# adwardlee/multitask-end-to-end-video-captioning

Hardware: AMD Instinct MI355X
Metric: sampled caption tokens/sec (REINFORCE step) (higher is better)
Workload: dtype f32

## Files before the change

### include/s2vt.h

```cpp
#ifndef S2VT_H
#define S2VT_H

#include <stddef.h>
#include <stdint.h>

#ifdef __cplusplus
extern "C" {
#endif

#define S2VT_OK 0
#define S2VT_E_BADARG (-1)
#define S2VT_E_ALIGN (-2)
#define S2VT_E_WORKSPACE (-3)
#define S2VT_E_HIP (-4)
#define S2VT_E_CHAIN_TIMEOUT (-5)

typedef void* s2vt_stream;

typedef struct s2vt_dims {
    int32_t dim_image;
    int32_t n_words;
    int32_t word_dim;
    int32_t lstm_dim;
    int32_t n_video_lstm_step;
// ... 236 lines not shown
int s2vt_cast_bf16_split(const float* src, int32_t ld, const int32_t* rowidx, int32_t R, int32_t C, int32_t transpose, uint16_t* dst,
                         uint16_t* dst_lo, int32_t ldd, int32_t Rp, float* colsum, uint16_t* row_dst, uint16_t* row_dst_lo, int32_t row_ldd,
                         void* scratch, size_t scratch_bytes, s2vt_stream stream);
int s2vt_gemm_bf16x3_nt(const uint16_t* Ah, const uint16_t* Al, int32_t lda, const uint16_t* Bh, const uint16_t* Bl, int32_t ldb, float* C,
                        int32_t ldc, int32_t M, int32_t N, int32_t Kp, int32_t accumulate, void* scratch, size_t scratch_bytes, s2vt_stream stream);
int s2vt_gemm_bf16x3_nt_tile(const uint16_t* Ah, const uint16_t* Al, int32_t lda, const uint16_t* Bh, const uint16_t* Bl, int32_t ldb, float* C,
                             int32_t ldc, int32_t M, int32_t N, int32_t Kp, int32_t accumulate, s2vt_stream stream, int32_t tile);
int s2vt_gemm_bf16x3_nt_tile_choice(int32_t M, int32_t N, int32_t cus);
int s2vt_gemm_bf16x1_nt(const uint16_t* Ah, int32_t lda, const uint16_t* Bh, int32_t ldb, float* C, int32_t ldc, int32_t M, int32_t N, int32_t Kp,
                        int32_t accumulate, s2vt_stream stream);

int s2vt_gemm_bf16x3_tn(const uint16_t* Ah, const uint16_t* Al, int32_t lda, const uint16_t* Bh, const uint16_t* Bl, int32_t ldb, float* C,
                        int32_t ldc, int32_t M, int32_t N, int32_t K, int32_t accumulate, float* bias, void* scratch, size_t scratch_bytes,
                        s2vt_stream stream);
int s2vt_split_grad_active(int32_t N);
int s2vt_split_grad_dlogits_planes(const s2vt_dims* d, int32_t B, int32_t N, size_t* hi_offset, size_t* lo_offset, int32_t* ld);
int s2vt_softmax_nll_fwd_bwd_split(float* logits, int32_t ld, int32_t R, int32_t V, const int32_t* target, const float* coef, float smoothing,
                                   const float* smoothing_rows, float* nll, float* lp_target, const s2vt_dims* d, int32_t B, int32_t N,
                                   void* split_ws, size_t split_ws_bytes, s2vt_stream stream);

int s2vt_gemm_bf16x3_nn(const uint16_t* Ah, const uint16_t* Al, int32_t lda, const uint16_t* Bh, const uint16_t* Bl, int32_t ldb, float* C,
                        int32_t ldc, int32_t M, int32_t N, int32_t K, int32_t accumulate, const float* bias, void* scratch, size_t scratch_bytes,
                        s2vt_stream stream);

int s2vt_split_fwd_stage(void);
int s2vt_split_fwd_active(int32_t N);
int s2vt_teacher_forced_fwd_split(const s2vt_dims* d, const s2vt_params* p, const float* video, int32_t B, int32_t N,
                                  const int32_t* caption, int32_t caption_steps, const int32_t* live_rows, int32_t n_live, float keep,
                                  uint64_t seed, const int32_t* video_id, const int32_t* sample_id, float* logits_out,
                                  void* workspace, size_t workspace_bytes, const void* sampler_workspace,
                                  size_t sampler_workspace_bytes, int32_t sampler_rows, void* split_ws, size_t split_ws_bytes,
                                  s2vt_stream stream);

int s2vt_bptt_dvideo(const s2vt_dims* d, const s2vt_params* p, int32_t B, int32_t N, float* d_video, void* workspace,
                      size_t workspace_bytes, s2vt_stream stream);

int s2vt_embed_scatter_add(const float* dE, int32_t ld, const int32_t* idx, int32_t R, int32_t E, float* dWemb,
                           s2vt_stream stream);
int s2vt_embed_scatter_add2(const float* dE, int32_t ld, const int32_t* idx_a, const int32_t* idx_b, float scale, int32_t R, int32_t E,
                            float* dWemb, s2vt_stream stream);
int s2vt_embed_scatter_addk(const float* dE, int32_t ld, const int32_t* ids, const float* w, int32_t k, int32_t R, int32_t E, float* dWemb,
                            s2vt_stream stream);

int s2vt_caption_mask(const int32_t* ids, int32_t N, int32_t Tc, float* mask, int32_t* target_tm, float* mask_sum, float* mask_sum_copy, s2vt_stream stream);
int s2vt_pg_coef(const float* mask, const float* rewards, const float* baseline, float scale, int32_t N, int32_t Tc, float* coef_tm,
                 s2vt_stream stream);
// ... 223 lines not shown
```

### multitask-end-to-end-video-captioning_amd/_lib.py

```python
from __future__ import annotations

import ctypes as C
import os

_HERE = os.path.dirname(os.path.abspath(__file__))
_LIB = None


class S2VTLibraryError(RuntimeError):
    pass


class S2VTChainTimeout(S2VTLibraryError):
    """A persistent recurrence (csrc/chain.hip) was starved of CUs and gave up a grid-wide wait (S2VT_E_CHAIN_TIMEOUT):
    activations computed since are suspect, variable updates queued behind it were skipped on the device.  Recover with
    Video_Caption_Generator.recover() (synchronise, acknowledge, fall back to per-step launches) and repeat the step."""


MODEL_RESIDUAL = 1


class Dims(C.Structure):
    _fields_ = [(n, C.c_int32) for n in ("dim_image", "n_words", "word_dim", "lstm_dim", "n_video_lstm_step",
                                         "n_caption_lstm_step", "label_dim", "reserved")]
# ... 99 lines not shown
    "s2vt_beam_workspace_bytes": (_sz, [_DP, _i32, _i32]),
    "s2vt_beam_encode": (C.c_int, [_DP, _PP, _vp, _i32, _i32, _vp, _sz, _vp]),
    "s2vt_beam_step": (C.c_int, [_DP, _PP, _i32, _i32, _i32, _i32, _vp, _vp, _vp, _i32, _vp, _vp, _vp, _vp, _sz, _vp]),
    "s2vt_train_workspace_bytes": (_sz, [_DP, _i32, _i32]),
    "s2vt_teacher_forced_fwd": (C.c_int, [_DP, _PP, _vp, _i32, _i32, _vp, _f32, _u64, _vp, _vp, _vp, _vp, _sz, _vp]),
    "s2vt_teacher_forced_fwd_reuse": (C.c_int, [_DP, _PP, _vp, _i32, _i32, _vp, _f32, _u64, _vp, _vp, _vp, _vp, _sz, _vp, _sz, _i32, _vp]),
    "s2vt_gemm_nt_splitk": (C.c_int, [_vp, _i32, _vp, _i32, _vp, _i32, _i32, _i32, _i32, _i32, _i32, _vp, _sz, _vp]),
    "s2vt_teacher_forced_fwd_steps": (C.c_int, [_DP, _PP, _vp, _i32, _i32, _vp, _i32, _f32, _u64, _vp, _vp, _vp, _vp, _sz, _vp, _sz, _i32, _vp]),
    "s2vt_teacher_forced_fwd_live": (C.c_int, [_DP, _PP, _vp, _i32, _i32, _vp, _i32, _vp, _i32, _f32, _u64, _vp, _vp, _vp, _vp, _sz, _vp, _sz, _i32, _vp]),
    "s2vt_bptt_bwd_live": (C.c_int, [_DP, _PP, _PP, _vp, _i32, _i32, _vp, _i32, _vp, _i32, _f32, _u64, _vp, _vp, _vp, _sz, _i32, _vp]),
    "s2vt_bf16_grad_workspace_bytes": (_sz, [_DP, _i32, _i32]),
    "s2vt_bptt_bwd_bf16": (C.c_int, [_DP, _PP, _PP, _vp, _i32, _i32, _vp, _i32, _vp, _i32, _f32, _u64, _vp, _vp, _vp, _sz, _i32, _vp, _sz, _vp]),
    "s2vt_cast_bf16": (C.c_int, [_vp, _i32, _vp, _i32, _i32, _i32, _vp, _i32, _i32, _vp, _vp, _i32, _vp, _sz, _vp]),
    "s2vt_gemm_bf16_nt": (C.c_int, [_vp, _i32, _vp, _i32, _vp, _i32, _i32, _i32, _i32, _i32, _i32, _vp]),
    "s2vt_split_grad_workspace_bytes": (_sz, [_DP, _i32, _i32]),
    "s2vt_bptt_bwd_split": (C.c_int, [_DP, _PP, _PP, _vp, _i32, _i32, _vp, _i32, _vp, _i32, _f32, _u64, _vp, _vp, _vp, _sz, _i32, _vp, _sz, _vp]),
    "s2vt_cast_bf16_split": (C.c_int, [_vp, _i32, _vp, _i32, _i32, _i32, _vp, _vp, _i32, _i32, _vp, _vp, _vp, _i32, _vp, _sz, _vp]),
    "s2vt_gemm_bf16x3_nt": (C.c_int, [_vp, _vp, _i32, _vp, _vp, _i32, _vp, _i32, _i32, _i32, _i32, _i32, _vp, _sz, _vp]),
    "s2vt_gemm_bf16x3_nt_tile": (C.c_int, [_vp, _vp, _i32, _vp, _vp, _i32, _vp, _i32, _i32, _i32, _i32, _i32, _vp, _i32]),
    "s2vt_gemm_bf16x3_nt_tile_choice": (C.c_int, [_i32, _i32, _i32]),
    "s2vt_gemm_bf16x1_nt": (C.c_int, [_vp, _i32, _vp, _i32, _vp, _i32, _i32, _i32, _i32, _i32, _vp]),
    "s2vt_gemm_bf16x3_tn": (C.c_int, [_vp, _vp, _i32, _vp, _vp, _i32, _vp, _i32, _i32, _i32, _i32, _i32, _vp, _vp, _sz, _vp]),
    "s2vt_gemm_bf16x3_nn": (C.c_int, [_vp, _vp, _i32, _vp, _vp, _i32, _vp, _i32, _i32, _i32, _i32, _i32, _vp, _vp, _sz, _vp]),
    "s2vt_split_grad_active": (C.c_int, [_i32]),
    "s2vt_split_fwd_stage": (C.c_int, []),
    "s2vt_split_fwd_active": (C.c_int, [_i32]),
    "s2vt_teacher_forced_fwd_split": (C.c_int, [_DP, _PP, _vp, _i32, _i32, _vp, _i32, _vp, _i32, _f32, _u64, _vp, _vp, _vp, _vp, _sz, _vp, _sz, _i32,
                                                _vp, _sz, _vp]),
    "s2vt_train_workspace_dz2": (C.c_int, [_DP, _i32, _i32, C.POINTER(_sz), C.POINTER(_sz)]),
    "s2vt_split_grad_dlogits_planes": (C.c_int, [_DP, _i32, _i32, C.POINTER(_sz), C.POINTER(_sz), C.POINTER(_i32)]),
    "s2vt_softmax_nll_fwd_bwd_split": (C.c_int, [_vp, _i32, _i32, _i32, _vp, _vp, _f32, _vp, _vp, _vp, _DP, _i32, _i32, _vp, _sz, _vp]),
    "s2vt_bptt_bwd_steps": (C.c_int, [_DP, _PP, _PP, _vp, _i32, _i32, _vp, _i32, _f32, _u64, _vp, _vp, _vp, _sz, _i32, _vp]),
    "s2vt_softmax_nll_fwd_bwd": (C.c_int, [_vp, _i32, _i32, _i32, _vp, _vp, _f32, _vp, _vp, _vp]),
    "s2vt_softmax_unshifted_argmax": (C.c_int, [_vp, _i32, _i32, _i32, _vp, _vp, _vp]),
    "s2vt_softmax_nll_fwd_bwd_rows": (C.c_int, [_vp, _i32, _i32, _i32, _vp, _vp, _vp, _vp, _vp, _vp]),
    "s2vt_bptt_bwd": (C.c_int, [_DP, _PP, _PP, _vp, _i32, _i32, _vp, _f32, _u64, _vp, _vp, _vp, _sz, _vp]),
    "s2vt_bptt_bwd_phase": (C.c_int, [_DP, _PP, _PP, _vp, _i32, _i32, _vp, _f32, _u64, _vp, _vp, _vp, _sz, _i32, _vp]),
    "s2vt_bptt_dvideo": (C.c_int, [_DP, _PP, _i32, _i32, _vp, _vp, _sz, _vp]),
    "s2vt_embed_scatter_add": (C.c_int, [_vp, _i32, _vp, _i32, _i32, _vp, _vp]),
    "s2vt_caption_mask": (C.c_int, [_vp, _i32, _i32, _vp, _vp, _vp, _vp, _vp]),
    "s2vt_pg_coef": (C.c_int, [_vp, _vp, _vp, _f32, _i32, _i32, _vp, _vp]),
    "s2vt_xe_prep": (C.c_int, [_vp, _vp, _i32, _i32, _f32, _f32, _i32, _vp, _vp, _vp, _vp]),
    "s2vt_mixed_prep": (C.c_int, [_vp, _vp, _vp, _vp, _vp, _vp, _i32, _i32, _i32, C.c_double, _f32, _i32, _f32, _f32, _vp, _vp, _vp, _vp, _vp, _vp]),
    "s2vt_mixed_loss": (C.c_int, [_vp, _vp, _vp, _i64, _i32, _i32, _vp, _vp]),
    "s2vt_step_scalars": (C.c_int, [_vp, _vp, _i64, _vp, _vp, _vp, _vp, _vp, _vp]),
    "s2vt_grad_finalize": (C.c_int, [_vp, _vp, _i64, _vp, _f32, _vp, _vp]),
# ... 127 lines not shown
```

### multitask-end-to-end-video-captioning_amd/csrc/bwd_bf16.hip

```cpp
#include <hip/hip_runtime.h>

#include <cstdlib>
#include <type_traits>

#include "internal.h"

namespace s2vt {
namespace {

typedef __bf16 bf16x8 __attribute__((ext_vector_type(8)));
typedef float f32x4 __attribute__((ext_vector_type(4)));
typedef float f32x16 __attribute__((ext_vector_type(16)));

template <bool SPLIT>
__global__ __launch_bounds__(256) void cast_rows_bf16_kernel(const float* __restrict__ src, int ld, const int32_t* __restrict__ rowidx,
                                                             int R, int K, uint16_t* __restrict__ dst, int ldd, int vec,
                                                             uint16_t* __restrict__ dst_lo, int ones, int width)
{
    const int cpr = width / 8;
    const long total = (long)R * cpr;
    for (long i = (long)blockIdx.x * 256 + threadIdx.x; i < total; i += (long)gridDim.x * 256) {
        const int r = (int)(i / cpr), k0 = (int)(i % cpr) * 8;
        const float* s = src + (size_t)(rowidx ? rowidx[r] : r) * ld + k0;
        float v[8];
// ... 196 lines not shown
                int row, col;
                if constexpr (MF == 16) {
                    row = m0 + wr * 64 + i * 16 + (lane >> 4) * 4 + e;
                    col = n0 + wc * 64 + j * 16 + (lane & 15);
                } else {
                    row = m0 + wr * 64 + i * 32 + (e & 3) + 8 * (e >> 2) + 4 * (lane >> 5);
                    col = n0 + wc * 64 + j * 32 + (lane & 31);
                }
                if (row < g.M && col < g.N) {
                    float* c = g.C + (size_t)row * g.ldc + col;
                    *c = g.accumulate ? *c + acc[i][j][e] : acc[i][j][e];
                }
            }
}


struct GemmX3Args {
    const uint16_t *Ah, *Al; int lda; const uint16_t *Bh, *Bl; int ldb; float* C; int ldc;
    int M, N, nk, nk_slab, accumulate, tiles_m, tiles_n;
    float* part;
    int K;
    float* bias; int Mo;
    const float* cbias;
};

enum : int { kX3NT = 0, kX3TN = 1, kX3NN = 2 };
enum : int { kX1NT = 3 };

constexpr int kX3BK = 32, kX3Slots = 4, kX3Plane = kTile * kX3BK;
constexpr int kX3TileM = 192, kX3TileN = 96;
constexpr int x3_lds_bytes(int tm, int tn) { return kX3Slots * 2 * (tm + tn) * kX3BK * 2; }
constexpr int x1_lds_bytes(int tm, int tn) { return kX3Slots * (tm + tn) * kX3BK * 2; }
constexpr int kX3Dma = kTile / 16;
typedef __attribute__((address_space(3))) void* x3_lds_ptr;
typedef short i16x4 __attribute__((ext_vector_type(4)));
typedef __attribute__((address_space(3))) i16x4* x3_tr_ptr;

template <int ND, int FORM = kX3NT>
__device__ __forceinline__ void x3_nt_loader(__amdgpu_buffer_rsrc_t rs, int r0, int rows, int ld, uint16_t* pdst, int slot_elems, int kbeg, int nk, int lane)
{
    static_assert(3 * ND < 64, "vmcnt is a 6-bit counter");
    uint32_t voff[ND];
    const int rr = lane >> 2, kg = (lane & 3) ^ ((rr >> 2) & 3);
#pragma unroll
    for (int b = 0; b < ND; ++b) {
        const int r = b * 16 + rr;
        voff[b] = r0 + r < rows ? (uint32_t)(r * ld + kg * 8) * 2u : kOob;
// ... 48 lines not shown
            const int p = w - 4;
            if constexpr (X1) {
                const int hr = (p < 2 ? BM : BN) / 2 * (p & 1);
                const int r0 = (p < 2 ? m0 : n0) + hr, rows = p < 2 ? g.M : g.N, ld = p < 2 ? g.lda : g.ldb;
                const __amdgpu_buffer_rsrc_t rs = __builtin_amdgcn_make_buffer_rsrc(const_cast<uint16_t*>((p < 2 ? g.Ah : g.Bh) + (size_t)min(r0, rows) * ld), 0, (int)kOob, 0x00020000);
                uint16_t* const pdst = x3lds + (p < 2 ? 0 : kPlaneA) + hr * kX3BK;
                if (p < 2) x3_nt_loader<BM / 32, kX1NT>(rs, r0, rows, ld, pdst, kSlot, kbeg, nk, lane);
                else x3_nt_loader<BN / 32, kX1NT>(rs, r0, rows, ld, pdst, kSlot, kbeg, nk, lane);
                return;
            } else {
                const uint16_t* const plane = p == 0 ? g.Ah : p == 1 ? g.Al : p == 2 ? g.Bh : g.Bl;
                const int r0 = p < 2 ? m0 : n0, rows = p < 2 ? g.M : g.N, ld = p < 2 ? g.lda : g.ldb;
                const __amdgpu_buffer_rsrc_t rs = __builtin_amdgcn_make_buffer_rsrc(const_cast<uint16_t*>(plane + (size_t)r0 * ld), 0, (int)kOob, 0x00020000);
                uint16_t* const pdst = x3lds + (p < 2 ? p * kPlaneA : 2 * kPlaneA + (p - 2) * kPlaneB);
                if (p < 2) x3_nt_loader<BM / 16>(rs, r0, rows, ld, pdst, kSlot, kbeg, nk, lane);
                else x3_nt_loader<BN / 16>(rs, r0, rows, ld, pdst, kSlot, kbeg, nk, lane);
                return;
            }
        }
    } else if (w >= 4) {
        const int p = w - 4;
        const bool TN = ATN == BTN ? ATN : p >= 2;
        const uint16_t* const plane = p == 0 ? g.Ah : p == 1 ? g.Al : p == 2 ? g.Bh : g.Bl;
        const int r0 = p < 2 ? m0 : n0, rows = p < 2 ? g.M : g.N, ld = p < 2 ? g.lda : g.ldb;
        const __amdgpu_buffer_rsrc_t rs = __builtin_amdgcn_make_buffer_rsrc(const_cast<uint16_t*>(plane + (TN ? (size_t)r0 : (size_t)r0 * ld)), 0,
                                                                            TN ? (int)(((uint32_t)g.K * (uint32_t)ld - (uint32_t)r0) * 2u) : (int)kOob, 0x00020000);
        uint32_t voff[kX3Dma];
        if (TN) {
            const int kr = lane >> 4, s = lane & 15;
#pragma unroll
            for (int b = 0; b < kX3Dma; ++b)
                voff[b] = (uint32_t)((b * 4 + kr) * ld + ((((s >> 1) ^ (kr | ((b & 2) << 1))) << 1) | (s & 1)) * 8) * 2u;
        } else {
            const int rr = lane >> 2, kg = (lane & 3) ^ ((rr >> 2) & 3);
#pragma unroll
            for (int b = 0; b < kX3Dma; ++b) {
                const int r = b * 16 + rr;
                voff[b] = r0 + r < rows ? (uint32_t)(r * ld + kg * 8) * 2u : kOob;
            }
        }
        auto issue = [&](int ks) __attribute__((always_inline)) {
            uint16_t* const dst = x3lds + ((ks % kX3Slots) * 4 + p) * kX3Plane;
            if (TN) {
                const uint32_t koff = (uint32_t)(kbeg + ks) * kX3BK * (uint32_t)ld * 2u;
#pragma unroll
                for (int b = 0; b < kX3Dma; ++b)
                    __builtin_amdgcn_raw_ptr_buffer_load_lds(rs, (x3_lds_ptr)(dst + b * 4 * kTile), 16, voff[b] + koff, 0, 0, 0);
            } else {
                const uint32_t soff = (uint32_t)(kbeg + ks) * kX3BK * 2u;
#pragma unroll
                for (int b = 0; b < kX3Dma; ++b)
                    __builtin_amdgcn_raw_ptr_buffer_load_lds(rs, (x3_lds_ptr)(dst + b * 16 * kX3BK), 16, voff[b], soff, 0, 0);
            }
        };
        auto wait_younger = [](int n) __attribute__((always_inline)) {
            if (n >= 2) wait_vmcnt<2 * kX3Dma>();
            else if (n == 1) wait_vmcnt<kX3Dma>();
            else wait_vmcnt<0>();
        };
        const int pro = min(kX3Slots, nk);
        for (int ks = 0; ks < pro; ++ks) issue(ks);
        if (pro - 1 >= 3) wait_vmcnt<3 * kX3Dma>();
        else wait_younger(pro - 1);
        asm volatile("" ::: "memory");
        __builtin_amdgcn_s_barrier();
        asm volatile("" ::: "memory");
        for (int k = 0; k < nk; ++k) {
            wait_younger(min(k + 3, nk - 1) - (k + 1));
            asm volatile("" ::: "memory");
            __builtin_amdgcn_s_barrier();
            asm volatile("" ::: "memory");
            if (k + kX3Slots < nk) issue(k + kX3Slots);
        }
        return;
    }

    const int wr = w >> 1, wc = w & 1;
    const int fofs = (lane & 15) * kX3BK + (((lane >> 4) ^ ((lane >> 2) & 3)) << 3);
    const int gq = lane >> 4, tq = (lane >> 2) & 3, tswz = tq | ((gq & 1) << 2);
    const int tofs = (gq * 8 + tq) * kTile + (lane & 3) * 4;
    f32x4 acc[FI][FJ];
#pragma unroll
    for (int i = 0; i < FI; ++i)
#pragma unroll
        for (int j = 0; j < FJ; ++j) acc[i][j] = f32x4{0.0f, 0.0f, 0.0f, 0.0f};
    constexpr int FX = FI > FJ ? FI : FJ, NPL = X1 ? 2 : 4;
    auto read = [&](int ks, bf16x8 (&f)[NPL][FX]) __attribute__((always_inline)) {
        const uint16_t* const s = x3lds + (ks % kX3Slots) * kSlot;
#pragma unroll
        for (int pl = 0; pl < NPL; ++pl)
#pragma unroll
            for (int i = 0; i < FX; ++i)
                if constexpr (X1) {
                    if (i < (pl == 0 ? FI : FJ))
                        f[pl][i] = *reinterpret_cast<const bf16x8*>(s + (pl == 0 ? wr * WM * kX3BK : kPlaneA + wc * WN * kX3BK) + i * 16 * kX3BK + fofs);
// ... 21 lines not shown
    };
    auto mul = [&](const bf16x8 (&f)[NPL][FX]) __attribute__((always_inline)) {
        if constexpr (X1) {
#pragma unroll
            for (int i = 0; i < FI; ++i)
#pragma unroll
                for (int j = 0; j < FJ; ++j) acc[i][j] = __builtin_amdgcn_mfma_f32_16x16x32_bf16(f[0][i], f[1][j], acc[i][j], 0, 0, 0);
        } else {
#pragma unroll
            for (int i = 0; i < FI; ++i)
#pragma unroll
                for (int j = 0; j < FJ; ++j) acc[i][j] = __builtin_amdgcn_mfma_f32_16x16x32_bf16(f[0][i], f[3][j], acc[i][j], 0, 0, 0);
#pragma unroll
            for (int i = 0; i < FI; ++i)
#pragma unroll
                for (int j = 0; j < FJ; ++j) acc[i][j] = __builtin_amdgcn_mfma_f32_16x16x32_bf16(f[1][i], f[2][j], acc[i][j], 0, 0, 0);
#pragma unroll
            for (int i = 0; i < FI; ++i)
#pragma unroll
                for (int j = 0; j < FJ; ++j) acc[i][j] = __builtin_amdgcn_mfma_f32_16x16x32_bf16(f[0][i], f[2][j], acc[i][j], 0, 0, 0);
        }
    };
    bf16x8 fa[NPL][FX], fb[NPL][FX];
    __syncthreads();
    if (nk > 0) read(0, fa);
    auto step = [&](int k, bf16x8 (&cur)[NPL][FX], bf16x8 (&nxt)[NPL][FX]) __attribute__((always_inline)) {
        asm volatile("s_waitcnt lgkmcnt(0)" ::: "memory");
        __syncthreads();
        if (k + 1 < nk) read(k + 1, nxt);
        mul(cur);
    };
    for (int k = 0; k < nk; k += 2) {
        step(k, fa, fb);
        step(k + 1, fb, fa);
    }
    float* const out = g.part ? g.part + (size_t)blockIdx.y * g.Mo * g.N : g.C;
    const int ldo = g.part ? g.N : g.ldc;
    const bool add = !g.part && g.accumulate;
#pragma unroll
    for (int i = 0; i < FI; ++i)
#pragma unroll
        for (int j = 0; j < FJ; ++j)
#pragma unroll
            for (int e = 0; e < 4; ++e) {
                const int row = m0 + wr * WM + i * 16 + (lane >> 4) * 4 + e, col = n0 + wc * WN + j * 16 + (lane & 15);
                if (row < g.M && col < g.N) {
                    float* c = out + (size_t)row * ldo + col;
                    if constexpr (FORM == kX3NN) {
                        const float v = !g.part && g.cbias ? acc[i][j][e] + g.cbias[col] : acc[i][j][e];
                        *c = add ? *c + v : v;
                    } else {
                        *c = add ? *c + acc[i][j][e] : acc[i][j][e];
                    }
                } else if (FORM == kX3TN && row == g.M && g.bias && col < g.N) {
                    if (g.part) out[(size_t)row * ldo + col] = acc[i][j][e];
                    else g.bias[col] += acc[i][j][e];
                }
            }
}

__global__ __launch_bounds__(256) void reduce_slabs_kernel(const float* __restrict__ part, int slabs, int M, int N, float* __restrict__ C, int ldc,
                                                           int accumulate, int Mo, float* __restrict__ bias, const float* __restrict__ cbias)
{
    const size_t MN = (size_t)Mo * N;
    for (size_t i = (size_t)blockIdx.x * 256 + threadIdx.x; i < MN; i += (size_t)gridDim.x * 256) {
        float s = part[i];
        for (int k = 1; k < slabs; ++k) s += part[(size_t)k * MN + i];
        const size_t r = i / N;
        if (r < (size_t)M) {
            float* c = C + r * ldc + i % N;
            if (cbias) s = s + cbias[i % N];
            *c = accumulate ? *c + s : s;
        } else {
            bias[i % N] += s;
        }
    }
}
}

hipError_t launch_cast_rows_bf16(const float* src, int ld, const int32_t* rowidx, int R, int K, uint16_t* dst, int ldd, hipStream_t st,
                                 uint16_t* dst_lo, int ones, int width)
// ... 65 lines not shown
    while (s < 8 && tiles * (s * 2) <= cus && nk / (s * 2) >= 16) s *= 2;
    return s;
}

int gemm_bf16x3_nt_tile_choice(int M, int N, int cus)
{
    const auto up = [](long long a, long long b) { return (a + b - 1) / b; };
    const long long t192 = up(M, kX3TileM) * up(N, kX3TileN), t128 = up(M, kTile) * up(N, kTile);
    return up(t192, cus) * (kX3TileM * kX3TileN) < up(t128, cus) * (kTile * kTile) ? 1 : 0;
}

int gemm_bf16x3_pick_tile(int M, int N)
{
    static const int knob = [] { const char* e = getenv("S2VT_PICK_TILE"); return e && (e[0] == '0' || e[0] == '1') && !e[1] ? e[0] - '0' : -1; }();
    return knob >= 0 ? knob : gemm_bf16x3_nt_tile_choice(M, N, x3_cus());
}

size_t gemm_bf16x3_part_floats(int M, int N, int Kp)
{
    const int s = gemm_bf16x3_slabs(M, N, Kp);
    return s > 1 ? (size_t)s * M * N : 0;
}

namespace {
template <int FORM, int BM = kTile, int BN = kTile>
hipError_t launch_x3(const uint16_t* Ah, const uint16_t* Al, int lda, const uint16_t* Bh, const uint16_t* Bl, int ldb, float* C, int ldc, int M, int N,
                     int Kp, int accumulate, float* bias, float* part, size_t part_floats, int cls, hipStream_t st, const float* cbias = nullptr)
{
    constexpr bool kWide = BM != BN, kOne = FORM == kX1NT;
    constexpr int kLds = kOne ? x1_lds_bytes(BM, BN) : x3_lds_bytes(BM, BN), kCfg = kOne ? 18 : kWide ? 17 : 16;
    if (M <= 0 || N <= 0) return hipSuccess;
    if (kWide && part) return hipErrorInvalidValue;
    static const hipError_t attr = hipFuncSetAttribute(reinterpret_cast<const void*>(gemm_bf16x3_kernel<FORM, BM, BN>), hipFuncAttributeMaxDynamicSharedMemorySize, kLds);
    if (attr != hipSuccess) return attr;
    GemmX3Args g;
    g.Ah = Ah; g.Al = Al; g.lda = lda; g.Bh = Bh; g.Bl = Bl; g.ldb = ldb; g.C = C; g.ldc = ldc; g.M = M; g.N = N;
    g.K = Kp; g.bias = bias; g.Mo = M + (bias ? 1 : 0); g.cbias = cbias;
    const int Kr = bf16_pad(Kp);
    g.nk = Kr / kX3BK; g.accumulate = accumulate;
    g.tiles_m = (g.Mo + BM - 1) / BM; g.tiles_n = (N + BN - 1) / BN;
    int slabs = part ? gemm_bf16x3_slabs(g.Mo, N, Kr) : 1;
    if ((size_t)slabs * g.Mo * N > part_floats) slabs = 1;
    g.nk_slab = ((g.nk + slabs - 1) / slabs + 1) & ~1;
    slabs = g.nk_slab ? (g.nk + g.nk_slab - 1) / g.nk_slab : 1;
    g.part = slabs > 1 ? part : nullptr;
    const dim3 grid((unsigned)(g.tiles_m * g.tiles_n), (unsigned)slabs);
    const bool prof = prof_wants(cls, kCfg);
    hipEvent_t e0 = nullptr, e1 = nullptr;
    if (prof) {
        hipError_t pe = prof_events(&e0, &e1);
        if (pe != hipSuccess) return pe;
        (void)hipEventRecord(e0, st);
    }
    hipLaunchKernelGGL((gemm_bf16x3_kernel<FORM, BM, BN>), grid, dim3(512), kLds, st, g);
    if (slabs > 1) {
        const size_t MN = (size_t)g.Mo * N, blocks = (MN + 255) / 256;
        hipLaunchKernelGGL(reduce_slabs_kernel, dim3((unsigned)(blocks < 4096 ? blocks : 4096)), dim3(256), 0, st, (const float*)part, slabs, M, N, C, ldc,
                           accumulate, g.Mo, bias, cbias);
    }
    if (prof) {
        (void)hipEventRecord(e1, st);
        const char* const name = kOne ? (cls == 2 ? "x1_192x96(dma) pick screen" : "x1_192x96(dma)")
                                 : kWide ? (cls == 2 ? "x3_192x96(dma) pick screen" : cls == 3 ? "x3_192x96(dma) wgrad" : "x3_192x96(dma) dgrad")
                                       : cls == 0 ? "x3_128x128(dma) fwd" : cls == 2 ? "x3_128x128(dma) pick screen" : cls == 3 ? "x3_128x128(dma) wgrad" : "x3_128x128(dma) dgrad";
        prof_record(cls, kCfg, name, 2.0 * M * (double)N * Kp, e0, e1);
    }
    return hipGetLastError();
}
}
// ... 11 lines not shown
    return launch_x3<kX1NT, kX3TileM, kX3TileN>(Ah, nullptr, lda, Bh, nullptr, ldb, C, ldc, M, N, Kp, accumulate, nullptr, nullptr, 0, cls, st);
}

bool gemm_bf16x3_tn_ok(int lda, int ldb, int K)
{
    const unsigned long long ld = (unsigned long long)(lda > ldb ? lda : ldb);
    return K >= 0 && lda > 0 && ldb > 0 && ((unsigned long long)bf16_pad(K) + 1) * ld * 2ull + 512ull < (1ull << 31);
}

hipError_t launch_gemm_bf16x3_tn(const uint16_t* Ah, const uint16_t* Al, int lda, const uint16_t* Bh, const uint16_t* Bl, int ldb, float* C, int ldc,
                                 int M, int N, int K, int accumulate, float* bias, float* part, size_t part_floats, int cls, hipStream_t st)
{
    if (!gemm_bf16x3_tn_ok(lda, ldb, K)) return hipErrorInvalidValue;
    return launch_x3<kX3TN>(Ah, Al, lda, Bh, Bl, ldb, C, ldc, M, N, K, accumulate, bias, part, part_floats, cls, st);
}

hipError_t launch_gemm_bf16x3_nn(const uint16_t* Ah, const uint16_t* Al, int lda, const uint16_t* Bh, const uint16_t* Bl, int ldb, float* C, int ldc,
                                 int M, int N, int K, int accumulate, const float* cbias, float* part, size_t part_floats, int cls, hipStream_t st)
{
    if (!gemm_bf16x3_tn_ok(ldb, ldb, K) || lda < bf16_pad(K) || (cbias && accumulate)) return hipErrorInvalidValue;
    return launch_x3<kX3NN>(Ah, Al, lda, Bh, Bl, ldb, C, ldc, M, N, K, accumulate, nullptr, part, part_floats, cls, st, cbias);
}

}
```

### multitask-end-to-end-video-captioning_amd/csrc/internal.h

```cpp
#pragma once
#include <hip/hip_runtime.h>
#include <stdint.h>

#include "gemm_mfma.h"

namespace s2vt {

hipError_t launch_gemm(const GemmArgs& a, int epi, int cfg, hipStream_t st);

struct ProfRow { int cls, cfg; long launches; double ms, flops; const char* name; };
void prof_enable(bool on);
bool prof_on();
bool prof_wants(int cls, int cfg);
void prof_filter(int cls, int cfg);
void prof_record(int cls, int cfg, const char* name, double flops, hipEvent_t e0, hipEvent_t e1);
hipError_t prof_events(hipEvent_t* e0, hipEvent_t* e1);
int prof_collect(ProfRow* rows, int max_rows);
int gemm_num_cfgs(int epi);
const char* gemm_cfg_name(int epi, int cfg);
struct GemmCfgInfo { const char* name; int BM, CG, fallback; bool has_scalar, has_live; };
bool gemm_cfg_info(int epi, int cfg, GemmCfgInfo* out);

struct TnArgs {
    const float* A; const int* rowidx; int lda;
// ... 261 lines not shown
struct CastTrArgs {
    const float* src; int ld; const int32_t* rowidx; int R, C;
    uint16_t* dst; int ldd; int Rp;
    float* colsum; float* part;
    uint16_t* rdst; int rldd;
    uint16_t* dst_lo; uint16_t* rdst_lo;
};
hipError_t launch_cast_tr_bf16(const CastTrArgs& a, hipStream_t st);
size_t cast_tr_part_floats(int Rp, int C);
hipError_t launch_gemm_bf16_nt(const uint16_t* A, int lda, const uint16_t* B, int ldb, float* C, int ldc, int M, int N, int Kp, int accumulate,
                               int mfma, hipStream_t st);
hipError_t launch_gemm_bf16x3_nt(const uint16_t* Ah, const uint16_t* Al, int lda, const uint16_t* Bh, const uint16_t* Bl, int ldb, float* C, int ldc,
                                 int M, int N, int Kp, int accumulate, float* part, size_t part_floats, int cls, hipStream_t st, int tile = 0);
int gemm_bf16x3_nt_tile_choice(int M, int N, int cus);
hipError_t launch_gemm_bf16x1_nt(const uint16_t* Ah, int lda, const uint16_t* Bh, int ldb, float* C, int ldc, int M, int N, int Kp, int accumulate, int cls,
                                 hipStream_t st);
int gemm_bf16x3_pick_tile(int M, int N);
size_t gemm_bf16x3_part_floats(int M, int N, int Kp);
bool gemm_bf16x3_tn_ok(int lda, int ldb, int K);
hipError_t launch_gemm_bf16x3_tn(const uint16_t* Ah, const uint16_t* Al, int lda, const uint16_t* Bh, const uint16_t* Bl, int ldb, float* C, int ldc,
                                 int M, int N, int K, int accumulate, float* bias, float* part, size_t part_floats, int cls, hipStream_t st);
hipError_t launch_gemm_bf16x3_nn(const uint16_t* Ah, const uint16_t* Al, int lda, const uint16_t* Bh, const uint16_t* Bl, int ldb, float* C, int ldc,
                                 int M, int N, int K, int accumulate, const float* cbias, float* part, size_t part_floats, int cls, hipStream_t st);
bool softmax_nll_split_ok(const float* logits, int ld, int V, const uint16_t* hi, const uint16_t* lo, int ldp);
hipError_t launch_softmax_nll_split(const float* logits, int ld, int R, int V, const int32_t* target, const float* coef, float smoothing, float* nll,
                                    float* lp_t, uint16_t* hi, uint16_t* lo, int ldp, hipStream_t st, const float* smooth_rows = nullptr);

int pick_screen_products();
constexpr int kPickScreenMaxH = 2048;
constexpr size_t kPickScreenHeadBytes = 256;
struct PickScreenWs {
    unsigned long long* counters;
    float* nwmax;
    uint16_t *Wh, *Wl;
    float* Wt;
    uint16_t *hh, *hl;
    float* L;
    int Hp, ldl, ldt;
};
hipError_t launch_pick_screen_prepare(const float* W, int H, int V, const PickScreenWs& s, hipStream_t st);
hipError_t launch_pick_screen_step(const float* h, int ldh, const float* W, const float* bias, int R, int H, int V, const int32_t* vid,
                                   const int32_t* sid, uint64_t seed, int step, unsigned long long* pick, int pick_stride, const PickScreenWs& s,
                                   hipStream_t st);

struct NnBwdArgs {
    const float* A; int lda;
// ... 9 lines not shown
```

### multitask-end-to-end-video-captioning_amd/csrc/train.hip

```cpp
#include <hip/hip_runtime.h>

#include <functional>
#include <mutex>

#include <cstdlib>

#include "api_util.h"

using namespace s2vt_api;

namespace s2vt_api {
SideStream& side_stream()
{
    constexpr int kMaxDev = 32;
    static SideStream table[kMaxDev];
    static bool made[kMaxDev] = {};
    static SideStream none;
    static const int mode = [] {
        const char* on = getenv("S2VT_OVERLAP");
        const int m = on ? atoi(on) : 2;
        return (m < 1 || m > 2) ? 0 : m;
    }();
    int dev = -1;
    if (mode == 0 || hipGetDevice(&dev) != hipSuccess || dev < 0 || dev >= kMaxDev) return none;
// ... 1617 lines not shown
    HIP_TRY(launch_gemm_bf16x1_nt(Ah, lda, Bh, ldb, C, ldc, M, N, Kp, accumulate, 3, S(stream)));
    return S2VT_OK;
}

int s2vt_gemm_bf16x3_nt_tile_choice(int32_t M, int32_t N, int32_t cus)
{
    if (M <= 0 || N <= 0 || cus <= 0) return S2VT_E_BADARG;
    return gemm_bf16x3_nt_tile_choice(M, N, cus);
}

int s2vt_gemm_bf16x3_nn(const uint16_t* Ah, const uint16_t* Al, int32_t lda, const uint16_t* Bh, const uint16_t* Bl, int32_t ldb, float* C,
                        int32_t ldc, int32_t M, int32_t N, int32_t K, int32_t accumulate, const float* bias, void* scratch, size_t scratch_bytes,
                        s2vt_stream stream)
{
    if (!Ah || !Al || !Bh || !Bl || !C || M < 0 || N < 0 || K < 0 || lda < bf16_pad(K) || ldb < N || ldc < N || (lda & 7) || (ldb & 7))
        return S2VT_E_BADARG;
    if (accumulate < 0 || accumulate > 1 || (bias && accumulate) || (scratch_bytes && !scratch) || !gemm_bf16x3_tn_ok(ldb, ldb, K)) return S2VT_E_BADARG;
    if ((reinterpret_cast<uintptr_t>(Ah) | reinterpret_cast<uintptr_t>(Al) | reinterpret_cast<uintptr_t>(Bh) | reinterpret_cast<uintptr_t>(Bl)) & 15)
        return S2VT_E_ALIGN;
    HIP_TRY(launch_gemm_bf16x3_nn(Ah, Al, lda, Bh, Bl, ldb, C, ldc, M, N, K, accumulate, bias, static_cast<float*>(scratch), scratch_bytes / 4, 0, S(stream)));
    return S2VT_OK;
}

int s2vt_cast_bf16(const float* src, int32_t ld, const int32_t* rowidx, int32_t R, int32_t C, int32_t transpose, uint16_t* dst, int32_t ldd,
                   int32_t Rp, float* colsum, uint16_t* row_dst, int32_t row_ldd, void* scratch, size_t scratch_bytes, s2vt_stream stream)
{
    if (!src || !dst || R < 0 || C <= 0 || ld < C || transpose < 0 || transpose > 1) return S2VT_E_BADARG;
    if (reinterpret_cast<uintptr_t>(dst) & 15) return S2VT_E_ALIGN;
    if (!transpose) {
        if (colsum || row_dst || ldd < bf16_pad(C) || (ldd & 7)) return S2VT_E_BADARG;
        HIP_TRY(launch_cast_rows_bf16(src, ld, rowidx, R, C, dst, ldd, S(stream)));
        return S2VT_OK;
    }
    if (Rp < R || Rp % kBf16K || ldd < Rp || (ldd & 7)) return S2VT_E_BADARG;
    if (row_dst && (row_ldd < bf16_pad(C) || (row_ldd & 3))) return S2VT_E_BADARG;
    if (row_dst && (reinterpret_cast<uintptr_t>(row_dst) & 7)) return S2VT_E_ALIGN;
    if (colsum && (!scratch || scratch_bytes < cast_tr_part_floats(Rp, C) * 4)) return S2VT_E_WORKSPACE;
    CastTrArgs a{src, ld, rowidx, R, C, dst, ldd, Rp, colsum, static_cast<float*>(scratch), row_dst, row_ldd};
    HIP_TRY(launch_cast_tr_bf16(a, S(stream)));
    return S2VT_OK;
}

int s2vt_gemm_bf16_nt(const uint16_t* A, int32_t lda, const uint16_t* Bm, int32_t ldb, float* C, int32_t ldc, int32_t M, int32_t N, int32_t Kp,
                      int32_t accumulate, int32_t mfma, s2vt_stream stream)
{
    if (!A || !Bm || !C || M < 0 || N < 0 || Kp < 0 || Kp % kBf16K || lda < Kp || ldb < Kp || ldc < N || (lda & 7) || (ldb & 7)) return S2VT_E_BADARG;
// ... 79 lines not shown
```

### multitask-end-to-end-video-captioning_amd/ops.py

```python
from __future__ import annotations

import ctypes as C

import torch

from . import _lib
from ._lib import AttnParams, Dims, Operand, Params, check, lib


def _stream():
    return C.c_void_p(torch.cuda.current_stream().cuda_stream)


def _ptr(t):
    return None if t is None else C.c_void_p(t.data_ptr())


def _chk_f32(*ts):
    for t in ts:
        if t is not None:
            assert t.is_cuda and t.dtype == torch.float32, "expected a CUDA float32 tensor"


def make_dims(dim_image, n_words, word_dim, lstm_dim, n_video_lstm_step, n_caption_lstm_step, label_dim=0, residual=False) -> Dims:
# ... 869 lines not shown
    scratch = workspace(32 * M * N, Ah.device, "gemm_bf16x3") if split_k and M * N else None
    check(lib().s2vt_gemm_bf16x3_nt(_ptr(Ah), _ptr(Al), Ah.stride(0), _ptr(Bh), _ptr(Bl), Bh.stride(0), _ptr(out), out.stride(0), M, N, Kp,
                                    int(bool(accumulate)), _ptr(scratch), 0 if scratch is None else scratch.numel(), _stream()),
          "s2vt_gemm_bf16x3_nt")
    return out


def gemm_bf16x3_nt_tile(Ah, Al, Bh, Bl, tile, out=None, accumulate=False):
    for t in (Ah, Al, Bh, Bl):
        assert t.is_cuda and t.dtype == torch.bfloat16 and t.stride(1) == 1
    assert Ah.shape == Al.shape and Bh.shape == Bl.shape and Ah.stride(0) == Al.stride(0) and Bh.stride(0) == Bl.stride(0)
    M, Kp = Ah.shape
    N = Bh.shape[0]
    if out is None:
        assert not accumulate
        out = torch.empty((M, N), dtype=torch.float32, device=Ah.device)
    _chk_f32(out)
    assert out.shape[0] == M and out.shape[1] == N and out.stride(1) == 1
    check(lib().s2vt_gemm_bf16x3_nt_tile(_ptr(Ah), _ptr(Al), Ah.stride(0), _ptr(Bh), _ptr(Bl), Bh.stride(0), _ptr(out), out.stride(0), M, N, Kp,
                                         int(bool(accumulate)), _stream(), int(tile)), "s2vt_gemm_bf16x3_nt_tile")
    return out


def gemm_bf16x1_nt(Ah, Bh, out=None, accumulate=False):
    for t in (Ah, Bh):
        assert t.is_cuda and t.dtype == torch.bfloat16 and t.stride(1) == 1
    M, Kp = Ah.shape
    N = Bh.shape[0]
    if out is None:
        assert not accumulate
        out = torch.empty((M, N), dtype=torch.float32, device=Ah.device)
    _chk_f32(out)
    assert out.shape[0] == M and out.shape[1] == N and out.stride(1) == 1
    check(lib().s2vt_gemm_bf16x1_nt(_ptr(Ah), Ah.stride(0), _ptr(Bh), Bh.stride(0), _ptr(out), out.stride(0), M, N, Kp, int(bool(accumulate)),
                                    _stream()), "s2vt_gemm_bf16x1_nt")
    return out


def gemm_bf16x3_nt_tile_choice(M, N, cus):
    r = lib().s2vt_gemm_bf16x3_nt_tile_choice(int(M), int(N), int(cus))
    if r < 0:
        check(r, "s2vt_gemm_bf16x3_nt_tile_choice")
    return r


def gemm_bf16_nt(A, B, out=None, accumulate=False, mfma=0, n=None):
# ... 671 lines not shown
```

Baseline: 792,500.

## Make bf16x3 square-tile GEMM persistent with a CU-sized grid and cross-tile pipelining

The square-tile bf16x3 GEMM kernel becomes persistent. When there are more tiles than CUs and split-K is off, it launches about one workgroup per CU (rounded to a multiple of 8), and each workgroup loops over several XCD-remapped tiles. The DMA producer warps prefetch across tile boundaries so the LDS pipeline does not drain between tiles, and the consumer resets its accumulators and writes output per tile. It is on by default and can be disabled with S2VT_X3_PERSIST=0; it adds an explicit-grid API and a plan helper. The aim is to remove wave-quantization tail effects and per-tile prologue and epilogue stalls, at the risk of load imbalance and more register pressure.

```diff
diff --git a/include/s2vt.h b/include/s2vt.h
--- a/include/s2vt.h
+++ b/include/s2vt.h
@@ -282,6 +282,11 @@
 int s2vt_gemm_bf16x3_nn(const uint16_t* Ah, const uint16_t* Al, int32_t lda, const uint16_t* Bh, const uint16_t* Bl, int32_t ldb, float* C,
                         int32_t ldc, int32_t M, int32_t N, int32_t K, int32_t accumulate, const float* bias, void* scratch, size_t scratch_bytes,
                         s2vt_stream stream);
+
+int s2vt_gemm_bf16x3_persistent(int32_t form, const uint16_t* Ah, const uint16_t* Al, int32_t lda, const uint16_t* Bh, const uint16_t* Bl, int32_t ldb,
+                                float* C, int32_t ldc, int32_t M, int32_t N, int32_t K, int32_t accumulate, float* bias, s2vt_stream stream,
+                                int32_t max_workgroups);
+int s2vt_gemm_bf16x3_persistent_plan(int32_t tiles_m, int32_t tiles_n, int32_t cus, int32_t workgroup, int32_t* tiles, int32_t cap, int32_t* count);
 
 int s2vt_split_fwd_stage(void);
 int s2vt_split_fwd_active(int32_t N);
diff --git a/multitask-end-to-end-video-captioning_amd/_lib.py b/multitask-end-to-end-video-captioning_amd/_lib.py
--- a/multitask-end-to-end-video-captioning_amd/_lib.py
+++ b/multitask-end-to-end-video-captioning_amd/_lib.py
@@ -145,6 +145,8 @@
     "s2vt_gemm_bf16x1_nt": (C.c_int, [_vp, _i32, _vp, _i32, _vp, _i32, _i32, _i32, _i32, _i32, _vp]),
     "s2vt_gemm_bf16x3_tn": (C.c_int, [_vp, _vp, _i32, _vp, _vp, _i32, _vp, _i32, _i32, _i32, _i32, _i32, _vp, _vp, _sz, _vp]),
     "s2vt_gemm_bf16x3_nn": (C.c_int, [_vp, _vp, _i32, _vp, _vp, _i32, _vp, _i32, _i32, _i32, _i32, _i32, _vp, _vp, _sz, _vp]),
+    "s2vt_gemm_bf16x3_persistent": (C.c_int, [_i32, _vp, _vp, _i32, _vp, _vp, _i32, _vp, _i32, _i32, _i32, _i32, _i32, _vp, _vp, _i32]),
+    "s2vt_gemm_bf16x3_persistent_plan": (C.c_int, [_i32, _i32, _i32, _i32, _vp, _i32, _vp]),
     "s2vt_split_grad_active": (C.c_int, [_i32]),
     "s2vt_split_fwd_stage": (C.c_int, []),
     "s2vt_split_fwd_active": (C.c_int, [_i32]),
diff --git a/multitask-end-to-end-video-captioning_amd/csrc/bwd_bf16.hip b/multitask-end-to-end-video-captioning_amd/csrc/bwd_bf16.hip
--- a/multitask-end-to-end-video-captioning_amd/csrc/bwd_bf16.hip
+++ b/multitask-end-to-end-video-captioning_amd/csrc/bwd_bf16.hip
@@ -242,7 +242,15 @@
     int K;
     float* bias; int Mo;
     const float* cbias;
+    int wgs;
 };
+
+__host__ __device__ inline int x3_remap(int orig, int nwg)
+{
+    const int xcd = orig & 7, q = nwg >> 3, rem = nwg & 7;
+    return (xcd < rem ? xcd * (q + 1) : rem * (q + 1) + (xcd - rem) * q) + (orig >> 3);
+}
+__host__ __device__ inline int x3_tiles_of(int b, int wgs, int nwg) { return b < nwg ? (nwg - 1 - b) / wgs + 1 : 0; }
 
 enum : int { kX3NT = 0, kX3TN = 1, kX3NN = 2 };
 enum : int { kX1NT = 3 };
@@ -337,25 +345,34 @@
         const int p = w - 4;
         const bool TN = ATN == BTN ? ATN : p >= 2;
         const uint16_t* const plane = p == 0 ? g.Ah : p == 1 ? g.Al : p == 2 ? g.Bh : g.Bl;
-        const int r0 = p < 2 ? m0 : n0, rows = p < 2 ? g.M : g.N, ld = p < 2 ? g.lda : g.ldb;
-        const __amdgpu_buffer_rsrc_t rs = __builtin_amdgcn_make_buffer_rsrc(const_cast<uint16_t*>(plane + (TN ? (size_t)r0 : (size_t)r0 * ld)), 0,
-                                                                            TN ? (int)(((uint32_t)g.K * (uint32_t)ld - (uint32_t)r0) * 2u) : (int)kOob, 0x00020000);
+        const int rows = p < 2 ? g.M : g.N, ld = p < 2 ? g.lda : g.ldb;
+        __amdgpu_buffer_rsrc_t rs;
         uint32_t voff[kX3Dma];
         if (TN) {
             const int kr = lane >> 4, s = lane & 15;
 #pragma unroll
             for (int b = 0; b < kX3Dma; ++b)
                 voff[b] = (uint32_t)((b * 4 + kr) * ld + ((((s >> 1) ^ (kr | ((b & 2) << 1))) << 1) | (s & 1)) * 8) * 2u;
-        } else {
-            const int rr = lane >> 2, kg = (lane & 3) ^ ((rr >> 2) & 3);
-#pragma unroll
-            for (int b = 0; b < kX3Dma; ++b) {
-                const int r = b * 16 + rr;
-                voff[b] = r0 + r < rows ? (uint32_t)(r * ld + kg * 8) * 2u : kOob;
-            }
-        }
-        auto issue = [&](int ks) __attribute__((always_inline)) {
-            uint16_t* const dst = x3lds + ((ks % kX3Slots) * 4 + p) * kX3Plane;
+        }
+        auto set_tile = [&](int t) __attribute__((always_inline)) {
+            const int wg = x3_remap(orig + t * g.wgs, nwg);
+            const int r0 = p < 2 ? (wg % g.tiles_m) * BM : (wg / g.tiles_m) * BN;
+            rs = __builtin_amdgcn_make_buffer_rsrc(const_cast<uint16_t*>(plane + (TN ? (size_t)r0 : (size_t)r0 * ld)), 0,
+                                                   TN ? (int)(((uint32_t)g.K * (uint32_t)ld - (uint32_t)r0) * 2u) : (int)kOob, 0x00020000);
+            if (!TN) {
+                const int rr = lane >> 2, kg = (lane & 3) ^ ((rr >> 2) & 3);
+#pragma unroll
+                for (int b = 0; b < kX3Dma; ++b) {
+                    const int r = b * 16 + rr;
+                    voff[b] = r0 + r < rows ? (uint32_t)(r * ld + kg * 8) * 2u : kOob;
+                }
+            }
+        };
+        const int T = x3_tiles_of(orig, g.wgs, nwg), S = T * nk;
+        int ct = 0, ck = 0, cs = 0;
+        if (T > 0) set_tile(0);
+        auto issue = [&](int ks, int slot) __attribute__((always_inline)) {
+            uint16_t* const dst = x3lds + (slot * 4 + p) * kX3Plane;
             if (TN) {
                 const uint32_t koff = (uint32_t)(kbeg + ks) * kX3BK * (uint32_t)ld * 2u;
 #pragma unroll
@@ -373,19 +390,27 @@
             else if (n == 1) wait_vmcnt<kX3Dma>();
             else wait_vmcnt<0>();
         };
-        const int pro = min(kX3Slots, nk);
-        for (int ks = 0; ks < pro; ++ks) issue(ks);
+        auto issue_next = [&]() __attribute__((always_inline)) {
+            issue(ck, cs % kX3Slots);
+            ++cs;
+            if (++ck == nk) {
+                ck = 0;
+                if (++ct < T) set_tile(ct);
+            }
+        };
+        const int pro = min(kX3Slots, S);
+        for (int i = 0; i < pro; ++i) issue_next();
         if (pro - 1 >= 3) wait_vmcnt<3 * kX3Dma>();
         else wait_younger(pro - 1);
         asm volatile("" ::: "memory");
         __builtin_amdgcn_s_barrier();
         asm volatile("" ::: "memory");
-        for (int k = 0; k < nk; ++k) {
-            wait_younger(min(k + 3, nk - 1) - (k + 1));
+        for (int s = 0; s < S; ++s) {
+            wait_younger(min(s + 3, S - 1) - (s + 1));
             asm volatile("" ::: "memory");
             __builtin_amdgcn_s_barrier();
             asm volatile("" ::: "memory");
-            if (k + kX3Slots < nk) issue(k + kX3Slots);
+            if (s + kX3Slots < S) issue_next();
         }
         return;
     }
@@ -453,41 +478,87 @@
         }
     };
     bf16x8 fa[NPL][FX], fb[NPL][FX];
-    __syncthreads();
-    if (nk > 0) read(0, fa);
-    auto step = [&](int k, bf16x8 (&cur)[NPL][FX], bf16x8 (&nxt)[NPL][FX]) __attribute__((always_inline)) {
-        asm volatile("s_waitcnt lgkmcnt(0)" ::: "memory");
+    if constexpr (BM != BN) {
         __syncthreads();
-        if (k + 1 < nk) read(k + 1, nxt);
-        mul(cur);
-    };
-    for (int k = 0; k < nk; k += 2) {
-        step(k, fa, fb);
-        step(k + 1, fb, fa);
-    }
-    float* const out = g.part ? g.part + (size_t)blockIdx.y * g.Mo * g.N : g.C;
-    const int ldo = g.part ? g.N : g.ldc;
-    const bool add = !g.part && g.accumulate;
-#pragma unroll
-    for (int i = 0; i < FI; ++i)
-#pragma unroll
-        for (int j = 0; j < FJ; ++j)
-#pragma unroll
-            for (int e = 0; e < 4; ++e) {
-                const int row = m0 + wr * WM + i * 16 + (lane >> 4) * 4 + e, col = n0 + wc * WN + j * 16 + (lane & 15);
-                if (row < g.M && col < g.N) {
-                    float* c = out + (size_t)row * ldo + col;
-                    if constexpr (FORM == kX3NN) {
-                        const float v = !g.part && g.cbias ? acc[i][j][e] + g.cbias[col] : acc[i][j][e];
-                        *c = add ? *c + v : v;
-                    } else {
+        if (nk > 0) read(0, fa);
+        auto step = [&](int k, bf16x8 (&cur)[NPL][FX], bf16x8 (&nxt)[NPL][FX]) __attribute__((always_inline)) {
+            asm volatile("s_waitcnt lgkmcnt(0)" ::: "memory");
+            __syncthreads();
+            if (k + 1 < nk) read(k + 1, nxt);
+            mul(cur);
+        };
+        for (int k = 0; k < nk; k += 2) {
+            step(k, fa, fb);
+            step(k + 1, fb, fa);
+        }
+        float* const out = g.part ? g.part + (size_t)blockIdx.y * g.Mo * g.N : g.C;
+        const int ldo = g.part ? g.N : g.ldc;
+        const bool add = !g.part && g.accumulate;
+#pragma unroll
+        for (int i = 0; i < FI; ++i)
+#pragma unroll
+            for (int j = 0; j < FJ; ++j)
+#pragma unroll
+                for (int e = 0; e < 4; ++e) {
+                    const int row = m0 + wr * WM + i * 16 + (lane >> 4) * 4 + e, col = n0 + wc * WN + j * 16 + (lane & 15);
+                    if (row < g.M && col < g.N) {
+                        float* c = out + (size_t)row * ldo + col;
                         *c = add ? *c + acc[i][j][e] : acc[i][j][e];
                     }
-                } else if (FORM == kX3TN && row == g.M && g.bias && col < g.N) {
-                    if (g.part) out[(size_t)row * ldo + col] = acc[i][j][e];
-                    else g.bias[col] += acc[i][j][e];
-                }
-            }
+                }
+    } else {
+        const int T = x3_tiles_of(orig, g.wgs, nwg), S = T * nk;
+        __syncthreads();
+        if (S > 0) read(0, fa);
+        auto step = [&](int s, bf16x8 (&cur)[NPL][FX], bf16x8 (&nxt)[NPL][FX]) __attribute__((always_inline)) {
+            asm volatile("s_waitcnt lgkmcnt(0)" ::: "memory");
+            __syncthreads();
+            if (s + 1 < S) read(s + 1, nxt);
+            mul(cur);
+        };
+        float* const out = g.part ? g.part + (size_t)blockIdx.y * g.Mo * g.N : g.C;
+        const int ldo = g.part ? g.N : g.ldc;
+        const bool add = !g.part && g.accumulate;
+        const bool usecb = FORM == kX3NN && !g.part && g.cbias;
+        for (int t = 0, s = 0; t < T; ++t) {
+            const int wg = t ? x3_remap(orig + t * g.wgs, nwg) : wgid;
+            const int tm0 = (wg % g.tiles_m) * BM, tn0 = (wg / g.tiles_m) * BN;
+            float cb[FJ];
+            if constexpr (FORM == kX3NN) {
+#pragma unroll
+                for (int j = 0; j < FJ; ++j) {
+                    const int col = tn0 + wc * WN + j * 16 + (lane & 15);
+                    cb[j] = usecb && col < g.N ? g.cbias[col] : 0.0f;
+                }
+            }
+            for (int k = 0; k < nk; k += 2, s += 2) {
+                step(s, fa, fb);
+                step(s + 1, fb, fa);
+            }
+#pragma unroll
+            for (int i = 0; i < FI; ++i)
+#pragma unroll
+                for (int j = 0; j < FJ; ++j) {
+#pragma unroll
+                    for (int e = 0; e < 4; ++e) {
+                        const int row = tm0 + wr * WM + i * 16 + (lane >> 4) * 4 + e, col = tn0 + wc * WN + j * 16 + (lane & 15);
+                        if (row < g.M && col < g.N) {
+                            float* c = out + (size_t)row * ldo + col;
+                            if constexpr (FORM == kX3NN) {
+                                const float v = usecb ? acc[i][j][e] + cb[j] : acc[i][j][e];
+                                *c = add ? *c + v : v;
+                            } else {
+                                *c = add ? *c + acc[i][j][e] : acc[i][j][e];
+                            }
+                        } else if (FORM == kX3TN && row == g.M && g.bias && col < g.N) {
+                            if (g.part) out[(size_t)row * ldo + col] = acc[i][j][e];
+                            else g.bias[col] += acc[i][j][e];
+                        }
+                    }
+                    acc[i][j] = f32x4{0.0f, 0.0f, 0.0f, 0.0f};
+                }
+        }
+    }
 }
 
 __global__ __launch_bounds__(256) void reduce_slabs_kernel(const float* __restrict__ part, int slabs, int M, int N, float* __restrict__ C, int ldc,
@@ -599,10 +670,31 @@
     return s > 1 ? (size_t)s * M * N : 0;
 }
 
+int gemm_bf16x3_persistent_grid(int tiles, int cus)
+{
+    if (tiles <= cus) return tiles;
+    const int g = cus & ~7;
+    return g > 8 ? g : 8;
+}
+
+int gemm_bf16x3_persistent_tiles(int tiles, int grid, int wg, int* out, int cap)
+{
+    const int n = x3_tiles_of(wg, grid, tiles);
+    for (int t = 0; t < n && t < cap; ++t) out[t] = x3_remap(wg + t * grid, tiles);
+    return n;
+}
+
+static bool x3_persist()
+{
+    static const bool on = [] { const char* e = getenv("S2VT_X3_PERSIST"); return !(e && e[0] == '0' && !e[1]); }();
+    return on;
+}
+
 namespace {
 template <int FORM, int BM = kTile, int BN = kTile>
 hipError_t launch_x3(const uint16_t* Ah, const uint16_t* Al, int lda, const uint16_t* Bh, const uint16_t* Bl, int ldb, float* C, int ldc, int M, int N,
-                     int Kp, int accumulate, float* bias, float* part, size_t part_floats, int cls, hipStream_t st, const float* cbias = nullptr)
+                     int Kp, int accumulate, float* bias, float* part, size_t part_floats, int cls, hipStream_t st, const float* cbias = nullptr,
+                     int max_wgs = 0)
 {
     constexpr bool kWide = BM != BN, kOne = FORM == kX1NT;
     constexpr int kLds = kOne ? x1_lds_bytes(BM, BN) : x3_lds_bytes(BM, BN), kCfg = kOne ? 18 : kWide ? 17 : 16;
@@ -621,7 +713,13 @@
     g.nk_slab = ((g.nk + slabs - 1) / slabs + 1) & ~1;
     slabs = g.nk_slab ? (g.nk + g.nk_slab - 1) / g.nk_slab : 1;
     g.part = slabs > 1 ? part : nullptr;
-    const dim3 grid((unsigned)(g.tiles_m * g.tiles_n), (unsigned)slabs);
+    const int tiles = g.tiles_m * g.tiles_n;
+    g.wgs = tiles;
+    if (!kWide && slabs == 1) {
+        if (max_wgs > 0) g.wgs = max_wgs < tiles ? max_wgs : tiles;
+        else if (x3_persist()) g.wgs = gemm_bf16x3_persistent_grid(tiles, x3_cus());
+    }
+    const dim3 grid((unsigned)g.wgs, (unsigned)slabs);
     const bool prof = prof_wants(cls, kCfg);
     hipEvent_t e0 = nullptr, e1 = nullptr;
     if (prof) {
@@ -679,4 +777,17 @@
     return launch_x3<kX3NN>(Ah, Al, lda, Bh, Bl, ldb, C, ldc, M, N, K, accumulate, nullptr, part, part_floats, cls, st, cbias);
 }
 
-}
+hipError_t launch_gemm_bf16x3_persistent(int form, const uint16_t* Ah, const uint16_t* Al, int lda, const uint16_t* Bh, const uint16_t* Bl, int ldb, float* C,
+                                         int ldc, int M, int N, int K, int accumulate, float* bias, int max_wgs, int cls, hipStream_t st)
+{
+    if (max_wgs < 1) return hipErrorInvalidValue;
+    if (form == kX3NT) return bias ? hipErrorInvalidValue : launch_x3<kX3NT>(Ah, Al, lda, Bh, Bl, ldb, C, ldc, M, N, K, accumulate, nullptr, nullptr, 0, cls, st, nullptr, max_wgs);
+    if (form == kX3TN) {
+        if (!gemm_bf16x3_tn_ok(lda, ldb, K)) return hipErrorInvalidValue;
+        return launch_x3<kX3TN>(Ah, Al, lda, Bh, Bl, ldb, C, ldc, M, N, K, accumulate, bias, nullptr, 0, cls, st, nullptr, max_wgs);
+    }
+    if (form != kX3NN || !gemm_bf16x3_tn_ok(ldb, ldb, K) || lda < bf16_pad(K) || (bias && accumulate)) return hipErrorInvalidValue;
+    return launch_x3<kX3NN>(Ah, Al, lda, Bh, Bl, ldb, C, ldc, M, N, K, accumulate, nullptr, nullptr, 0, cls, st, bias, max_wgs);
+}
+
+}
diff --git a/multitask-end-to-end-video-captioning_amd/csrc/internal.h b/multitask-end-to-end-video-captioning_amd/csrc/internal.h
--- a/multitask-end-to-end-video-captioning_amd/csrc/internal.h
+++ b/multitask-end-to-end-video-captioning_amd/csrc/internal.h
@@ -307,6 +307,10 @@
                                  int M, int N, int K, int accumulate, float* bias, float* part, size_t part_floats, int cls, hipStream_t st);
 hipError_t launch_gemm_bf16x3_nn(const uint16_t* Ah, const uint16_t* Al, int lda, const uint16_t* Bh, const uint16_t* Bl, int ldb, float* C, int ldc,
                                  int M, int N, int K, int accumulate, const float* cbias, float* part, size_t part_floats, int cls, hipStream_t st);
+int gemm_bf16x3_persistent_grid(int tiles, int cus);
+int gemm_bf16x3_persistent_tiles(int tiles, int grid, int wg, int* out, int cap);
+hipError_t launch_gemm_bf16x3_persistent(int form, const uint16_t* Ah, const uint16_t* Al, int lda, const uint16_t* Bh, const uint16_t* Bl, int ldb, float* C,
+                                         int ldc, int M, int N, int K, int accumulate, float* bias, int max_wgs, int cls, hipStream_t st);
 bool softmax_nll_split_ok(const float* logits, int ld, int V, const uint16_t* hi, const uint16_t* lo, int ldp);
 hipError_t launch_softmax_nll_split(const float* logits, int ld, int R, int V, const int32_t* target, const float* coef, float smoothing, float* nll,
                                     float* lp_t, uint16_t* hi, uint16_t* lo, int ldp, hipStream_t st, const float* smooth_rows = nullptr);
diff --git a/multitask-end-to-end-video-captioning_amd/csrc/train.hip b/multitask-end-to-end-video-captioning_amd/csrc/train.hip
--- a/multitask-end-to-end-video-captioning_amd/csrc/train.hip
+++ b/multitask-end-to-end-video-captioning_amd/csrc/train.hip
@@ -1663,6 +1663,31 @@
     return S2VT_OK;
 }
 
+int s2vt_gemm_bf16x3_persistent(int32_t form, const uint16_t* Ah, const uint16_t* Al, int32_t lda, const uint16_t* Bh, const uint16_t* Bl, int32_t ldb,
+                                float* C, int32_t ldc, int32_t M, int32_t N, int32_t K, int32_t accumulate, float* bias, s2vt_stream stream,
+                                int32_t max_workgroups)
+{
+    if (form < 0 || form > 2 || max_workgroups < 1) return S2VT_E_BADARG;
+    if (!Ah || !Al || !Bh || !Bl || !C || M < 0 || N < 0 || K < 0 || ldc < N || (lda & 7) || (ldb & 7) || accumulate < 0 || accumulate > 1) return S2VT_E_BADARG;
+    if (form == 0 && (K % kBf16K || lda < K || ldb < K || bias)) return S2VT_E_BADARG;
+    if (form == 1 && (lda < M + (bias ? 1 : 0) || ldb < N || !gemm_bf16x3_tn_ok(lda, ldb, K))) return S2VT_E_BADARG;
+    if (form == 2 && (lda < bf16_pad(K) || ldb < N || (bias && accumulate) || !gemm_bf16x3_tn_ok(ldb, ldb, K))) return S2VT_E_BADARG;
+    if ((reinterpret_cast<uintptr_t>(Ah) | reinterpret_cast<uintptr_t>(Al) | reinterpret_cast<uintptr_t>(Bh) | reinterpret_cast<uintptr_t>(Bl)) & 15)
+        return S2VT_E_ALIGN;
+    HIP_TRY(launch_gemm_bf16x3_persistent(form, Ah, Al, lda, Bh, Bl, ldb, C, ldc, M, N, K, accumulate, bias, max_workgroups, form == 2 ? 0 : 3, S(stream)));
+    return S2VT_OK;
+}
+
+int s2vt_gemm_bf16x3_persistent_plan(int32_t tiles_m, int32_t tiles_n, int32_t cus, int32_t workgroup, int32_t* tiles, int32_t cap, int32_t* count)
+{
+    if (tiles_m <= 0 || tiles_n <= 0 || cus <= 0 || (int64_t)tiles_m * tiles_n > (1 << 24)) return S2VT_E_BADARG;
+    const int n = tiles_m * tiles_n, grid = gemm_bf16x3_persistent_grid(n, cus);
+    if (!tiles && !count) return grid;
+    if (!tiles || !count || cap < 0 || workgroup < 0 || workgroup >= grid) return S2VT_E_BADARG;
+    *count = gemm_bf16x3_persistent_tiles(n, grid, workgroup, tiles, cap);
+    return grid;
+}
+
 int s2vt_cast_bf16(const float* src, int32_t ld, const int32_t* rowidx, int32_t R, int32_t C, int32_t transpose, uint16_t* dst, int32_t ldd,
                    int32_t Rp, float* colsum, uint16_t* row_dst, int32_t row_ldd, void* scratch, size_t scratch_bytes, s2vt_stream stream)
 {
diff --git a/multitask-end-to-end-video-captioning_amd/ops.py b/multitask-end-to-end-video-captioning_amd/ops.py
--- a/multitask-end-to-end-video-captioning_amd/ops.py
+++ b/multitask-end-to-end-video-captioning_amd/ops.py
@@ -915,6 +915,51 @@
     return out
 
 
+X3_FORMS = {"nt": 0, "tn": 1, "nn": 2}
+
+
+def gemm_bf16x3_persistent(form, Ah, Al, Bh, Bl, max_workgroups, M=None, N=None, K=None, out=None, accumulate=False, bias=None):
+    for t in (Ah, Al, Bh, Bl):
+        assert t.is_cuda and t.dtype == torch.bfloat16 and t.stride(1) == 1
+    assert Ah.shape == Al.shape and Bh.shape == Bl.shape and Ah.stride(0) == Al.stride(0) and Bh.stride(0) == Bl.stride(0)
+    f = X3_FORMS[form]
+    if f == 0:
+        M, K, N = Ah.shape[0], Ah.shape[1], Bh.shape[0]
+    elif f == 1:
+        K = Ah.shape[0]
+        M = Ah.shape[1] if M is None else int(M)
+        N = Bh.shape[1] if N is None else int(N)
+    else:
+        M = Ah.shape[0]
+        K = Bh.shape[0] if K is None else int(K)
+        N = Bh.shape[1] if N is None else int(N)
+    if out is None:
+        assert not accumulate
+        out = torch.empty((M, N), dtype=torch.float32, device=Ah.device)
+    _chk_f32(out, bias)
+    assert out.shape[0] == M and out.shape[1] == N and out.stride(1) == 1
+    check(lib().s2vt_gemm_bf16x3_persistent(f, _ptr(Ah), _ptr(Al), Ah.stride(0), _ptr(Bh), _ptr(Bl), Bh.stride(0), _ptr(out), out.stride(0), M, N, K,
+                                            int(bool(accumulate)), _ptr(bias), _stream(), int(max_workgroups)), "s2vt_gemm_bf16x3_persistent")
+    return out
+
+
+def gemm_bf16x3_persistent_plan(tiles_m, tiles_n, cus, workgroup=None):
+    import ctypes
+    L = lib()
+    if workgroup is None:
+        grid = L.s2vt_gemm_bf16x3_persistent_plan(int(tiles_m), int(tiles_n), int(cus), 0, None, 0, None)
+        if grid < 0:
+            check(grid, "s2vt_gemm_bf16x3_persistent_plan")
+        return grid
+    cap = int(tiles_m) * int(tiles_n)
+    buf = (ctypes.c_int32 * max(cap, 1))()
+    cnt = ctypes.c_int32(0)
+    grid = L.s2vt_gemm_bf16x3_persistent_plan(int(tiles_m), int(tiles_n), int(cus), int(workgroup), buf, cap, ctypes.byref(cnt))
+    if grid < 0:
+        check(grid, "s2vt_gemm_bf16x3_persistent_plan")
+    return grid, list(buf[:cnt.value])
+
+
 def gemm_bf16x1_nt(Ah, Bh, out=None, accumulate=False):
     for t in (Ah, Bh):
         assert t.is_cuda and t.dtype == torch.bfloat16 and t.stride(1) == 1
```

Result: no change. 800,300, median of 6 (+1.0%).
